# VictoriaMetrics/VictoriaLogs

Hardware: NVIDIA H100
Metric: log rows scanned/sec (LogsQL phrase+regex) (higher is better)
Workload: dtype u8

## Files before the change

### victorialogs_b200/csrc/vl_engine.cu

```cuda
#include <dlfcn.h>
#include <algorithm>
#include <atomic>
#include <chrono>
#include <cmath>
#include <limits>
#include <thread>
#include <cstdio>
#include <cstdlib>
#include <cstring>
#include <functional>
#include <map>
#include <memory>
#include <mutex>
#include "vl_copier.h"
#include "vl_engine.h"
#include "vl_kernels.cuh"
#include "vl_program.h"
#include "vl_part.h"
#include "vl_mathnum.cuh"

using namespace vl;

namespace vl {
static thread_local std::string g_thread_err;
// ... 47 lines not shown
}

namespace {

struct ZstdWriter {
    size_t (*compress)(void*, size_t, const void*, size_t, int) = nullptr;
    size_t (*bound)(size_t) = nullptr;
    unsigned (*is_error)(size_t) = nullptr;
    bool ok = false;
    ZstdWriter() {
        void* h = dlopen("libzstd.so.1", RTLD_NOW | RTLD_GLOBAL);
        if (!h) return;
        compress = (decltype(compress))dlsym(h, "ZSTD_compress");
        bound = (decltype(bound))dlsym(h, "ZSTD_compressBound");
        is_error = (decltype(is_error))dlsym(h, "ZSTD_isError");
        ok = compress && bound && is_error;
    }
};
ZstdWriter& zstd_writer() { static ZstdWriter z; return z; }

}

namespace vl {
void finish_batch_layout(vlscan_ctx* ctx, vlscan_batch* b, const std::vector<uint32_t>& rows) {
    b->nblocks = rows.size();
    b->h_rows = rows;
    b->h_word_off.assign(rows.size() + 1, 0);
    b->rows = 0;
    for (size_t i = 0; i < rows.size(); i++) { b->h_word_off[i + 1] = b->h_word_off[i] + (rows[i] + 63) / 64; b->rows += rows[i]; }
    b->nwords = b->h_word_off.back();
    std::vector<uint32_t> wb(b->nwords);
    std::vector<uint64_t> init(b->nwords);
    for (size_t i = 0; i < rows.size(); i++) {
        for (uint64_t w = b->h_word_off[i]; w < b->h_word_off[i + 1]; w++) { wb[w] = (uint32_t)i; init[w] = ~0ull; }
        uint32_t tail = rows[i] & 63;
        if (tail) init[b->h_word_off[i + 1] - 1] = (~0ull) >> (64 - tail);
    }
    b->blk_rows.ensure(std::max<size_t>(rows.size() * 4, 16));
    b->blk_word_off.ensure((rows.size() + 1) * 8);
    b->word_block.ensure(std::max<size_t>(b->nwords * 4, 16));
    b->init_bitmap.ensure(std::max<size_t>(b->nwords * 8, 16));
    if (!rows.empty()) VL_CUDA(cudaMemcpyAsync(b->blk_rows.p, rows.data(), rows.size() * 4, cudaMemcpyHostToDevice, ctx->stream));
    VL_CUDA(cudaMemcpyAsync(b->blk_word_off.p, b->h_word_off.data(), (rows.size() + 1) * 8, cudaMemcpyHostToDevice, ctx->stream));
    if (b->nwords) {
        VL_CUDA(cudaMemcpyAsync(b->word_block.p, wb.data(), b->nwords * 4, cudaMemcpyHostToDevice, ctx->stream));
        VL_CUDA(cudaMemcpyAsync(b->init_bitmap.p, init.data(), b->nwords * 8, cudaMemcpyHostToDevice, ctx->stream));
    }
    VL_CUDA(cudaStreamSynchronize(ctx->stream));
}
}

static uint64_t collect_values_blocks(const vlscan_block* blocks, uint64_t nblocks, std::vector<ZValuesBlock>& zv, const uint8_t* need = nullptr, uint32_t nfields = 0, std::vector<size_t>* at = nullptr) {
    uint64_t zc = 512;
    if (at) at->assign((size_t)nblocks * nfields, SIZE_MAX);
    for (uint64_t b = 0; b < nblocks; b++)
        for (uint32_t k = 0; k < blocks[b].ncols; k++) {
            const vlscan_column& c = blocks[b].cols[k];
            if (c.kind != VLSCAN_COL_VALUES || c.stage != VLSCAN_STAGE_ONDISK) continue;
            if (need && (c.field >= nfields || !need[b * nfields + c.field])) continue;
            if (at && c.field < nfields && (*at)[b * nfields + c.field] == SIZE_MAX) (*at)[b * nfields + c.field] = zv.size();
            zv.push_back({c.values, (size_t)c.values_len, zc});
            zc += c.values_len;
        }
    return zc;
}
static double now_s() { return std::chrono::duration<double>(std::chrono::steady_clock::now().time_since_epoch()).count(); }

namespace {
struct Upload {
    vlscan_ctx* ctx; vlscan_batch* out; const vlscan_block* blocks; uint64_t nblocks; uint32_t nfields; vlscan_stats* stats;
    const std::vector<char>* need_bloom;
    std::vector<DevColumn>& cols = out->h_cols;
    const bool dbg = getenv("VLSCAN_DEBUG_TIMING") != nullptr; const double t_start = now_s();
    Copier io{ctx};
    std::vector<uint32_t> rows = std::vector<uint32_t>(nblocks);
    std::vector<Piece> pieces;
    std::vector<std::unique_ptr<std::vector<uint8_t>>> owned;
    uint64_t cursor = 16;
    ZstdJob zjob;
    uint64_t regen_cursor = 0;
    struct Ondisk { uint64_t col; uint32_t lens_frame, data_frame; uint64_t lens_rel, data_rel; };
    std::vector<Ondisk> ondisk;
    std::vector<OndiskCol> ocols;
    struct TsFrame { uint64_t block; uint32_t frame; uint64_t rel; };
    std::vector<TsFrame> ts_frames;
    std::vector<DevTimestamps> tsv;
    std::vector<ZValuesBlock> zv; std::vector<ZValuesInfo> zinfo; std::vector<size_t> zv_of; std::vector<uint64_t> ts_zoff; size_t zbad = SIZE_MAX; std::string zmsg;
    uint64_t add_piece(const uint8_t* src, uint64_t len) { uint64_t off = arena_reserve(cursor, len); if (len) pieces.push_back({src, len, off}); return off; }
    template <class F> void walk(bool ts, F&& f) {
        for (uint64_t b = 0; b < nblocks; b++) {
            const vlscan_block& blk = blocks[b];
            if (blk.rows > (8u << 20)) throw BadInput("block rows exceed maxRowsPerBlock (8Mi)");
            rows[b] = (uint32_t)blk.rows;
            if (ts) timestamps(blk, b);
            for (uint32_t k = 0; k < blk.ncols; k++) {
                if (blk.cols[k].field >= nfields) throw BadInput("column refers to a field outside the batch field table");
                f(blk, blk.cols[k], (size_t)b * nfields + blk.cols[k].field);
            }
        }
    }
    void sources(const uint8_t* need, bool ts) {
        uint64_t zc = collect_values_blocks(blocks, nblocks, zv, need, nfields, &zv_of);
        for (const ZValuesBlock& v : zv) if (v.n) io.src.push_back({v.p, v.n, v.zoff});
        ts_zoff.resize(ts ? nblocks : 0);
        for (uint64_t b = 0; b < nblocks && ts; b++) {
            const vlscan_block& blk = blocks[b];
            if (blk.ts_marshal_type != MT_ZSTD_NEAREST_DELTA2 && blk.ts_marshal_type != MT_ZSTD_NEAREST_DELTA) continue;
            if (blk.timestamps_len > vl::part::kMaxTimestampsBlockSize) throw BadInput("timestamps block size cannot exceed 8 MiB");
            ts_zoff[b] = zc;
            if (blk.timestamps_len) io.src.push_back({blk.timestamps, blk.timestamps_len, zc});
            zc += blk.timestamps_len;
        }
        if (!io.src.empty()) { ctx->zsrc.ensure(zc + 512); io.send_sources(ctx->zsrc.as<uint8_t>()); }
        zinfo.resize(zv.size());
        const double t_w = now_s();
        if (!zv.empty()) zjob.add_values_blocks(zv.data(), zv.size(), host_threads(), zinfo.data(), &zbad, &zmsg);
        if (dbg) fprintf(stderr, "[vlscan upload] header walk of %zu values blocks on %d host threads: %.1f ms (after %.1f ms of collecting and enqueueing the copies)\n",
                         zv.size(), host_threads(), 1e3 * (now_s() - t_w), 1e3 * (t_w - t_start));
    }
    template <class F> void header(const vlscan_column& c, size_t i, F&& payload) {
        DevColumn& d = cols[i];
        if (d.kind != COL_MISSING) throw BadInput("duplicate column for one field in a block");
        if (c.kind == VLSCAN_COL_CONST) {
            d.kind = COL_CONST; d.meta_len = (uint32_t)c.const_len; d.meta_off = add_piece(c.const_value, c.const_len);
            return;
        }
        if (c.kind != VLSCAN_COL_VALUES) throw BadInput("unknown column kind");
        if (c.value_type < VT_STRING || c.value_type >= VT_MAX) throw BadInput("unknown valueType");
        d.kind = COL_VALUES; d.vt = c.value_type; d.min_value = c.min_value; d.max_value = c.max_value;
        payload();
        if (c.bloom_len % 8) throw BadInput("cannot unmarshal bloomFilter from src with size not multiple by 8");
        if (need_bloom && !(*need_bloom)[c.field]) { d.bloom_words = 0; d.bloom_off = add_piece(c.bloom, 0); }
        else { d.bloom_words = (uint32_t)(c.bloom_len / 8); d.bloom_off = add_piece(c.bloom, c.bloom_len); }
        if (c.value_type == VT_DICT) {
            if (c.dict_len > 8) throw BadInput("valuesDict may contain max 8 items");
            d.dict_len = c.dict_len;
            uint32_t total = c.dict_len ? c.dict_offsets[c.dict_len] : 0;
            d.meta_len = total;
            if (c.dict_len && c.dict_blob == (const uint8_t*)c.dict_offsets + 4 * (c.dict_len + 1)) {
// ... 34 lines not shown
            d.data_const = (blk.rows >= 2 && lt >= 4 && data_len == d.lens_const) ? 1 : 0;
        } else throw BadInput("unknown values stage");
    }
    void timestamps(const vlscan_block& blk, uint64_t b) {
        if (!blk.ts_marshal_type) return;
        if (blk.ts_marshal_type > MT_NEAREST_DELTA) throw BadInput("unknown MarshalType of a timestamps block");
        if (blk.timestamps_len > vl::part::kMaxTimestampsBlockSize) throw BadInput("timestamps block size cannot exceed 8 MiB");
        if (tsv.empty()) { tsv.resize(nblocks); memset(tsv.data(), 0, nblocks * sizeof(DevTimestamps)); }
        DevTimestamps& t = tsv[b];
        t.first = blk.min_timestamp; t.max = blk.max_timestamp;
        if (blk.ts_marshal_type == MT_ZSTD_NEAREST_DELTA2 || blk.ts_marshal_type == MT_ZSTD_NEAREST_DELTA) {
            uint64_t regen = 0; uint32_t id = 0;
            zjob.add_frame(blk.timestamps, blk.timestamps_len, ts_zoff[b], &regen, &id);
            if (regen > 10ull * blk.rows + 16) throw BadInput("cannot unmarshal timestamps: the decompressed block is larger than its varints can be");
            t.mt = blk.ts_marshal_type == MT_ZSTD_NEAREST_DELTA2 ? MT_NEAREST_DELTA2 : MT_NEAREST_DELTA;
            t.len = (uint32_t)regen;
            ts_frames.push_back({b, id, arena_reserve(regen_cursor, regen)});
        } else {
            t.mt = (uint8_t)blk.ts_marshal_type; t.len = (uint32_t)blk.timestamps_len;
            t.off = add_piece(blk.timestamps, blk.timestamps_len);
        }
    }

    uint64_t commit(DevBuf& region, const std::vector<uint64_t>* patch, bool layout) {
        const uint64_t regen_base = (cursor + kArenaAlign - 1) / kArenaAlign * kArenaAlign;
        for (const Ondisk& o : ondisk) {
            DevColumn& d = cols[o.col];
            d.lens_off += regen_base; d.data_off += regen_base;
            zjob.set_dst(o.lens_frame, regen_base + o.lens_rel); zjob.set_dst(o.data_frame, regen_base + o.data_rel);
        }
        for (const TsFrame& tf : ts_frames) { tsv[tf.block].off = regen_base + tf.rel; zjob.set_dst(tf.frame, regen_base + tf.rel); }
        const bool have_z = !ondisk.empty() || !ts_frames.empty();
        if (have_z) cursor = regen_base + regen_cursor;
        const uint64_t bytes = cursor + kArenaPad;
        const double t_desc = now_s();
        region.ensure(bytes);
        const double t_alloc = now_s();
        uint8_t* cols_base = region.as<uint8_t>();
        std::vector<ColPatch> patches;
        if (patch) {
            const uint64_t delta = (uint64_t)(uintptr_t)region.p - (uint64_t)(uintptr_t)out->arena.p;
            cols_base = out->arena.as<uint8_t>();
            patches.resize(patch->size());
            for (size_t i = 0; i < patch->size(); i++) {
                DevColumn& d = cols[(*patch)[i]];
                d.lens_off += delta; d.data_off += delta;
                patches[i].col = (*patch)[i]; patches[i].c = d;
            }
        }
        cudaStream_t cs = ctx->copy_stream;
        cudaEvent_t ev_cleared = io.events.make(), ev_copied = io.events.make();
        VL_CUDA(cudaMemsetAsync(region.p, 0, bytes, ctx->stream));
        VL_CUDA(cudaEventRecord(ev_cleared, ctx->stream));
        VL_CUDA(cudaStreamWaitEvent(cs, ev_cleared, 0));
        const double t_h2d = dbg ? now_s() : 0;
        double t_zrun = 0;
        if (have_z) {
            zjob.set_group_hook([&](uint64_t src_end) { io.wait_sources(ctx->stream, src_end); });
            zjob.run(ctx, ctx->zsrc.as<uint8_t>(), region.as<uint8_t>());
            io.ship_sources(UINT64_MAX);
            if (dbg) t_zrun = now_s();
        }
        io.copy(pieces, region.as<uint8_t>());
        DevBuf& table = patch ? ctx->patch : out->cols;
        const void* entries = patch ? (const void*)patches.data() : (const void*)cols.data();
        const size_t table_bytes = patch ? patches.size() * sizeof(ColPatch) : cols.size() * sizeof(DevColumn);
        table.ensure(std::max<size_t>(table_bytes, 16));
        if (table_bytes) VL_CUDA(cudaMemcpyAsync(table.p, entries, table_bytes, cudaMemcpyHostToDevice, cs));
        io.h2d += table_bytes;
        if (!patch) out->has_ts = !tsv.empty();
        if (!tsv.empty()) {
            out->ts.ensure(nblocks * sizeof(DevTimestamps));
            VL_CUDA(cudaMemcpyAsync(out->ts.p, tsv.data(), nblocks * sizeof(DevTimestamps), cudaMemcpyHostToDevice, cs));
            io.h2d += nblocks * sizeof(DevTimestamps);
        }
        VL_CUDA(cudaEventRecord(ev_copied, cs));
        if (!patches.empty()) {
            VL_CUDA(cudaStreamWaitEvent(ctx->stream, ev_copied, 0));
            k_patch_cols<<<cdiv(patches.size(), 128), 128, 0, ctx->stream>>>(out->cols.as<DevColumn>(), ctx->patch.as<ColPatch>(), (uint32_t)patches.size());
            launch_check(ctx);
        }
        const double t_enq = dbg ? now_s() : 0;
        if (have_z) {
            VL_CUDA(cudaStreamWaitEvent(ctx->stream, ev_copied, 0));
            ctx->zcols.ensure(16 + ocols.size() * sizeof(OndiskCol));
            VL_CUDA(cudaMemsetAsync(ctx->zcols.p, 0, 16, ctx->stream));
            VL_CUDA(cudaMemcpyAsync(ctx->zcols.as<uint8_t>() + 16, ocols.data(), ocols.size() * sizeof(OndiskCol), cudaMemcpyHostToDevice, ctx->stream));
            if (!ocols.empty()) {
                k_finish_ondisk_cols<<<cdiv(ocols.size(), 128), 128, 0, ctx->stream>>>(cols_base, out->cols.as<DevColumn>(), (const OndiskCol*)(ctx->zcols.as<uint8_t>() + 16),
                                                                                         (uint32_t)ocols.size(), ctx->zcols.as<unsigned long long>());
                launch_check(ctx);
            }
            io.h2d += ocols.size() * sizeof(OndiskCol);
            zjob.check(ctx);
            unsigned long long cst[2] = {0, 0};
            VL_CUDA(cudaMemcpy(cst, ctx->zcols.p, 16, cudaMemcpyDeviceToHost));
            static const char* what[] = {"", "cannot unmarshal uint64 block type from empty src", "unexpected uint64 block type", "unexpected block length for uint items", "row length does not fit 32 bits"};
            if (cst[0]) throw BadInput(what[std::min<unsigned long long>(cst[0], 4)]);
        }
        VL_CUDA(cudaStreamWaitEvent(ctx->stream, ev_copied, 0));
        double t_copy = 0;
        if (dbg) { VL_CUDA(cudaStreamSynchronize(ctx->stream)); t_copy = now_s(); }
        if (nfields) out->note_columns(cols);
        if (layout) finish_batch_layout(ctx, out, rows);
        else VL_CUDA(cudaStreamSynchronize(ctx->stream));
        if (dbg) fprintf(stderr, "[vlscan upload] blocks=%llu arena=%.1f MB h2d=%.1f MB pieces=%zu+%zu pinned=%d: describe %.1f ms, alloc %.1f ms, copy %.1f ms (%.1f GB/s), "
                                 "zstd %llu frames / %llu blocks / %llu sequences: enqueue %.1f ms, decode %.1f ms; layout %.1f ms\n", (unsigned long long)nblocks,
                         bytes / 1e6, io.h2d / 1e6, pieces.size(), io.src.size(), (int)io.all_pinned, 1e3 * (t_desc - t_start), 1e3 * (t_alloc - t_desc), 1e3 * (t_enq - (t_zrun > 0 ? t_zrun : t_h2d)), io.h2d / 1e9 / std::max(t_copy - t_start, 1e-9),
                         (unsigned long long)zjob.frames(), (unsigned long long)zjob.compressed_blocks(), (unsigned long long)zjob.sequences(), 1e3 * (t_zrun > 0 ? t_zrun - t_h2d : 0), 1e3 * (t_copy - t_enq), 1e3 * (now_s() - t_copy));
        if (layout) io.h2d += out->nwords * 12 + nblocks * 12;
        if (stats) stats->h2d_bytes += io.h2d;
        return bytes;
    }
};
}

enum UploadMode { UP_FULL = 0, UP_HEADERS = 1, UP_VALUES = 2, UP_LATE = 3 };
static void do_upload(vlscan_ctx* ctx, const char* const* field_names, const size_t* field_name_lens, uint32_t nfields, const vlscan_block* blocks,
                      uint64_t nblocks, vlscan_batch* out, vlscan_stats* stats, const std::vector<char>* need_bloom = nullptr, UploadMode mode = UP_FULL,
                      const uint8_t* need = nullptr, uint64_t* zframes = nullptr) {
    VL_CUDA(cudaSetDevice(ctx->device));
    if (nblocks > 0xFFFFFFF0ull) throw BadInput("too many blocks in one batch");
    out->device = ctx->device; out->nfields = nfields;
    Upload u{ctx, out, blocks, nblocks, nfields, stats, need_bloom};
    if (mode == UP_FULL || mode == UP_HEADERS) {
        for (uint32_t f = 0; f < nfields; f++) out->field_names.emplace_back(field_names[f], field_name_lens[f]);
        u.cols.assign((size_t)nblocks * std::max<uint32_t>(nfields, 1), DevColumn{});
        memset(u.cols.data(), 0, u.cols.size() * sizeof(DevColumn));
        out->late_used = 0; out->split_hdr = mode == UP_HEADERS;
    } else if (u.cols.size() != (size_t)nblocks * std::max<uint32_t>(nfields, 1) || !need) throw BadInput("internal: values phase of a bloom-first upload without its header phase");
    try {
        switch (mode) {
        case UP_FULL:
            u.sources(nullptr, true);
            u.walk(true, [&](const vlscan_block& blk, const vlscan_column& c, size_t i) { u.header(c, i, [&] { u.values(blk, c, i); }); });
            out->arena_bytes = u.commit(out->arena, nullptr, true);
            out->harena_bytes = 0;
            std::vector<DevColumn>().swap(out->h_cols);
            break;
        case UP_HEADERS:
            u.walk(false, [&](const vlscan_block&, const vlscan_column& c, size_t i) {
                u.header(c, i, [&] {
                    if (c.stage != VLSCAN_STAGE_ONDISK && c.stage != VLSCAN_STAGE_DECODED) throw BadInput("unknown values stage");
                    u.cols[i].values_state = VALUES_DEFERRED;
                });
            });
            out->harena_bytes = u.commit(out->harena, nullptr, true);
            break;
        case UP_VALUES:
            u.sources(need, true);
            u.walk(true, [&](const vlscan_block& blk, const vlscan_column& c, size_t i) {
                if (c.kind != VLSCAN_COL_VALUES) return;
                u.cols[i].values_state = need[i] ? VALUES_STAGED : VALUES_ABSENT;
                if (need[i]) u.values(blk, c, i);
            });
            out->arena_bytes = u.commit(out->arena, nullptr, false);
            break;
        case UP_LATE: {
            std::vector<uint64_t> staged;
            u.sources(need, false);
            u.walk(false, [&](const vlscan_block& blk, const vlscan_column& c, size_t i) {
                if (c.kind != VLSCAN_COL_VALUES || !need[i]) return;
                if (u.cols[i].values_state == VALUES_STAGED) throw BadInput("duplicate column for one field in a block");
                u.cols[i].values_state = VALUES_STAGED;
                u.values(blk, c, i);
                staged.push_back(i);
            });
            if (out->late_used == out->late.size()) out->late.emplace_back();
            u.commit(out->late[out->late_used], &staged, false);
            out->late_used++;
            *zframes += u.zjob.frames();
            break;
        }
        }
    } catch (...) {
        cudaStreamSynchronize(ctx->copy_stream); cudaStreamSynchronize(ctx->stream);
        throw;
    }
}

const uint32_t* vl::row_offsets(vlscan_ctx* ctx, const BatchView& B, int slot, const uint32_t* list, const uint32_t* wc, unsigned long long* stats, int wc_slot) {
    uint8_t* ready = ctx->ready[slot].as<uint8_t>();
    if (!ctx->ready_cleared[slot]) { VL_CUDA(cudaMemsetAsync(ready, 0, B.nblocks, ctx->stream)); ctx->ready_cleared[slot] = 1; }
    k_lens_offsets<<<ctx->sm_count * 8, 256, 0, ctx->stream>>>(B, slot, list, wc, ctx->row_off8[slot].as<uint32_t>(), ready, stats, wc_slot); launch_check(ctx);
    return ctx->row_off8[slot].as<uint32_t>();
}

namespace {
struct ScanRun {
    vlscan_ctx* ctx; const vlscan_program* prog; const vlscan_batch* batch;
    DevProgram P; BatchView B; std::vector<int> field_slot;
    unsigned long long* stats;
    size_t regs_used = 0;

    uint64_t* new_reg() {
        if (regs_used == ctx->regs.size()) ctx->regs.emplace_back();
        DevBuf& r = ctx->regs[regs_used++];
        r.ensure(std::max<size_t>(B.nwords * 8, 16));
        return r.as<uint64_t>();
    }
    void free_reg() { regs_used--; }
    void copy_reg(uint64_t* dst, const uint64_t* src) { if (B.nwords) VL_CUDA(cudaMemcpyAsync(dst, src, B.nwords * 8, cudaMemcpyDeviceToDevice, ctx->stream)); }
// ... 873 lines not shown
```

### victorialogs_b200/csrc/vl_zstd.cu

```cuda
#include "vl_zstd.h"

#include <algorithm>
#include <array>
#include <atomic>
#include <chrono>
#include <cstdio>
#include <cstdlib>
#include <cstring>
#include <exception>
#include <thread>

#include "vl_engine.h"
#include "vl_zstd.cuh"
#include "vl_zstd_job.h"

namespace vl {

using namespace zs;

struct ZstdDev {
    DevBuf frames, blocks, bstate, huf_tab, fse_tab, huf_state, fse_state, predef, lits, seqs, frame_err, status, lists;
    bool predef_ready = false;
    cudaStream_t xstream = nullptr;
    std::vector<cudaEvent_t> events;
    cudaEvent_t event(size_t i) {
        while (events.size() <= i) { cudaEvent_t e; VL_CUDA(cudaEventCreateWithFlags(&e, cudaEventDisableTiming)); events.push_back(e); }
        return events[i];
    }
    void* hpin = nullptr; size_t hpin_cap = 0;
    void* ensure_hpin(size_t n) {
        if (n <= hpin_cap) return hpin;
        if (hpin) cudaFreeHost(hpin);
        hpin = nullptr; hpin_cap = 0;
        VL_CUDA(cudaMallocHost(&hpin, n + n / 4 + 4096)); hpin_cap = n + n / 4 + 4096;
        return hpin;
    }
    void release() {
        DevBuf* all[] = {&frames, &blocks, &bstate, &huf_tab, &fse_tab, &huf_state, &fse_state, &predef, &lits, &seqs, &frame_err, &status, &lists};
        for (DevBuf* b : all) b->release();
        for (cudaEvent_t e : events) cudaEventDestroy(e);
        events.clear();
        if (xstream) cudaStreamDestroy(xstream);
        xstream = nullptr;
        if (hpin) cudaFreeHost(hpin);
        hpin = nullptr; hpin_cap = 0;
    }
};

static __global__ void k_pull_words(uint4* __restrict__ dst, const uint4* __restrict__ src, size_t n) {
    for (size_t i = (size_t)blockIdx.x * blockDim.x + threadIdx.x; i < n; i += (size_t)gridDim.x * blockDim.x) dst[i] = src[i];
}
void zstd_dev_free(ZstdDev* d) { if (d) { d->release(); delete d; } }

namespace {
inline unsigned cdiv_u(uint64_t a, uint64_t b) { return (unsigned)((a + b - 1) / b); }
}

struct ZstdJob::Impl : ZstdJobImpl {};

ZstdJob::ZstdJob() : m(new Impl) {}
ZstdJob::~ZstdJob() { delete m; }
bool ZstdJob::empty() const { return m->frames.empty(); }
uint64_t ZstdJob::frames() const { return m->frames.size(); }
uint64_t ZstdJob::blocks() const { return m->blocks.size(); }
uint64_t ZstdJob::compressed_blocks() const { return m->n_compressed; }
uint64_t ZstdJob::sequences() const { return m->n_seqs; }
// ... 31 lines not shown
                dry.add_bytes_block(v[i].p + c1, v[i].n - c1, v[i].zoff + c1, &r, &id);
            } catch (const BadInput&) { break; }
        }
        total_seqs = dry.m->n_seqs;
    }
    auto taper = [&] { if (!group_scale_env()) m->limit_scale = (m->groups.empty() || m->n_seqs > total_seqs - total_seqs / 12) ? 1 : 4; };
    for (size_t i = 0; i < n; i++) {
        try {
            uint32_t f1 = 0, f2 = 0;
            taper();
            const size_t c1 = add_bytes_block(v[i].p, v[i].n, v[i].zoff, &info[i].lens_len, &f1);
            taper();
            const size_t c2 = add_bytes_block(v[i].p + c1, v[i].n - c1, v[i].zoff + c1, &info[i].data_len, &f2);
            if (c1 + c2 != v[i].n) throw BadInput("unexpected non-empty tail after reading bytes block with strings");
        } catch (const BadInput& e) { *bad = i; *msg = e.msg; return; }
    }
    if (!group_scale_env()) m->limit_scale = 1;
}

void ZstdJob::prepare() { m->prepare(); }

void ZstdJob::digest(uint64_t out[4]) const { m->digest(out); }

void ZstdJob::run(vlscan_ctx* ctx, const uint8_t* zsrc, uint8_t* arena) {
    Impl& J = *m;
    if (J.frames.empty()) return;
    auto now = [] { return std::chrono::duration<double>(std::chrono::steady_clock::now().time_since_epoch()).count(); };
    const double t_prep = now();
    J.prepare();
    const double t_lists = now();
    const std::vector<uint32_t>& lists = J.lists;
    if (!ctx->zdev) ctx->zdev = new ZstdDev;
    ZstdDev& D = *ctx->zdev;
    cudaStream_t st = ctx->stream;
    D.frames.ensure(J.frames.size() * sizeof(ZFrame) + 16); D.blocks.ensure(J.blocks.size() * sizeof(ZBlock) + 16); D.bstate.ensure(J.blocks.size() * sizeof(ZBlockState));
    D.frame_err.ensure(J.frames.size() * 4); D.status.ensure(16); D.lists.ensure(lists.size() * 4 + 16);
    D.huf_tab.ensure(std::max<size_t>((size_t)J.max_huf * Z_HUF_TABLE * 2, 16)); D.huf_state.ensure(std::max<size_t>((size_t)J.max_huf * sizeof(ZSlotState), 16));
    D.fse_tab.ensure(std::max<size_t>((size_t)J.max_fse * Z_FSE_SLOT_BYTES, 16)); D.fse_state.ensure(std::max<size_t>((size_t)J.max_fse * sizeof(ZSlotState), 16));
    const size_t lits_stride = (J.max_lits + 64 + 255) / 256 * 256, seqs_stride = std::max<size_t>(J.max_seqs, 1);
    D.lits.ensure(2 * lits_stride); D.seqs.ensure(2 * seqs_stride * 16);
    if (!D.xstream) VL_CUDA(cudaStreamCreateWithFlags(&D.xstream, cudaStreamNonBlocking));
    if (!D.predef_ready) {
        D.predef.ensure(Z_FSE_SLOT_BYTES);
        k_zstd_predef<<<1, 32, 0, st>>>(D.predef.as<uint8_t>());
        VL_CUDA(cudaFuncSetAttribute(k_seq_decode, cudaFuncAttributeMaxDynamicSharedMemorySize, (int)(Z_SEQ_CTA_LANES * (Z_FSE_SLOT_BYTES + Z_LINEBUF))));
        VL_CUDA(cudaFuncSetAttribute(k_huf_decode, cudaFuncAttributeMaxDynamicSharedMemorySize, (int)(Z_HUF_CTA_BLOCKS * Z_HUF_TABLE * 2)));
        ctx->launches++; VL_CUDA(cudaGetLastError());
        D.predef_ready = true;
    }
    {
        auto up16 = [](size_t n) { return (n + 15) / 16 * 16; };
        const size_t nf = up16(J.frames.size() * sizeof(ZFrame)), nb = up16(J.blocks.size() * sizeof(ZBlock)), nl = up16(lists.size() * 4);
        uint8_t* h = (uint8_t*)D.ensure_hpin(nf + nb + nl + 64);
        const double t_cp = now();
        J.spread_copy(h, J.frames.data(), J.frames.size() * sizeof(ZFrame));
        J.spread_copy(h + nf, J.blocks.data(), J.blocks.size() * sizeof(ZBlock));
        if (!lists.empty()) J.spread_copy(h + nf + nb, lists.data(), lists.size() * 4);
        if (getenv("VLSCAN_DEBUG_TIMING")) fprintf(stderr, "[vlscan zstd] host: work lists of %zu launch groups %.1f ms, %.1f MB of tables to pinned memory %.1f ms (%d threads)\n",
                                                   J.groups.size(), 1e3 * (t_lists - t_prep), (nf + nb + nl) / 1e6, 1e3 * (now() - t_cp), std::max(J.threads, 1));
        k_pull_words<<<296, 256, 0, st>>>(D.frames.as<uint4>(), (const uint4*)h, nf / 16); ctx->launches++;
        k_pull_words<<<296, 256, 0, st>>>(D.blocks.as<uint4>(), (const uint4*)(h + nf), nb / 16); ctx->launches++;
        if (nl) { k_pull_words<<<296, 256, 0, st>>>(D.lists.as<uint4>(), (const uint4*)(h + nf + nb), nl / 16); ctx->launches++; }
        VL_CUDA(cudaGetLastError());
    }
    VL_CUDA(cudaMemsetAsync(D.frame_err.p, 0, J.frames.size() * 4, st));
    VL_CUDA(cudaMemsetAsync(D.status.p, 0, 16, st));
    VL_CUDA(cudaMemsetAsync(D.bstate.p, 0, J.blocks.size() * sizeof(ZBlockState), st));
    ZView V{};
    V.src = zsrc; V.arena = arena; V.frames = D.frames.as<ZFrame>(); V.blocks = D.blocks.as<ZBlock>(); V.bstate = D.bstate.as<ZBlockState>();
    V.huf_tab = D.huf_tab.as<uint16_t>(); V.fse_tab = D.fse_tab.as<uint8_t>(); V.huf_state = D.huf_state.as<ZSlotState>(); V.fse_state = D.fse_state.as<ZSlotState>();
    V.predef = D.predef.as<uint8_t>(); V.lits = D.lits.as<uint8_t>(); V.seqs = D.seqs.as<uint4>(); V.frame_err = D.frame_err.as<unsigned int>();
    V.status = D.status.as<unsigned long long>();
    const uint32_t* L = D.lists.as<uint32_t>();
    const bool dbg = getenv("VLSCAN_DEBUG_TIMING") != nullptr;
    static const char* phase_name[6] = {"huf_build", "huf_decode", "fse_build", "seq_decode", "seq_resolve", "execute"};
    std::vector<std::pair<int, std::pair<cudaEvent_t, cudaEvent_t>>> marks;
    int phase = 0;
    static const bool overlap = [] { const char* e = getenv("VLSCAN_ZSTD_OVERLAP"); return !e || atoi(e) != 0; }();
    cudaStream_t xs = overlap ? D.xstream : st;
    cudaStream_t cur_stream = st;
    auto begin = [&](int p) { phase = p; if (dbg) { cudaEvent_t a, b; cudaEventCreate(&a); cudaEventCreate(&b); cudaEventRecord(a, cur_stream); marks.push_back({p, {a, b}}); } };
    auto launched = [&] { ctx->launches++; VL_CUDA(cudaGetLastError()); if (dbg) cudaEventRecord(marks.back().second.second, cur_stream); };
    VL_CUDA(cudaEventRecord(D.event(0), st)); VL_CUDA(cudaStreamWaitEvent(xs, D.event(0), 0));
    size_t gi = 0;
    for (const Group& g : J.groups) {
        uint32_t nh = g.huf_hi - g.huf_lo, nl = g.lit_hi - g.lit_lo, ns = g.seq_hi - g.seq_lo, nf = g.frame_hi - g.frame_lo;
        if (J.group_hook) {
            uint64_t need = 0;
            for (uint32_t i = J.frames[g.frame_lo].blk_lo; i < J.frames[g.frame_hi - 1].blk_hi; i++) need = std::max<uint64_t>(need, J.blocks[i].src + (J.blocks[i].type == ZB_RLE ? 1 : J.blocks[i].size));
            J.group_hook(need);
        }
        ZView W = V;
        W.lits = V.lits + (gi & 1) * lits_stride; W.seqs = V.seqs + (gi & 1) * seqs_stride;
        cudaEvent_t ev_entropy = D.event(1 + 2 * gi), ev_exec = D.event(2 + 2 * gi);
        cur_stream = st;
// ... 6 lines not shown
        }
        VL_CUDA(cudaEventRecord(ev_entropy, st));
        VL_CUDA(cudaStreamWaitEvent(xs, ev_entropy, 0));
        cur_stream = xs;
        begin(4); k_seq_resolve<<<cdiv_u(nf, 64), 64, 0, xs>>>(W, g.frame_lo, nf); launched();
        begin(5); k_execute<<<cdiv_u((uint64_t)nf * 32, Z_EXEC_WARPS * 32), Z_EXEC_WARPS * 32, 0, xs>>>(W, L + g.ord_lo, nf); launched();
        VL_CUDA(cudaEventRecord(ev_exec, xs));
        gi++;
    }
    if (gi) VL_CUDA(cudaStreamWaitEvent(st, D.event(2 + 2 * (gi - 1)), 0));
    cur_stream = st;
    if (dbg) {
        VL_CUDA(cudaStreamSynchronize(xs)); VL_CUDA(cudaStreamSynchronize(st));
        float tot[6] = {0, 0, 0, 0, 0, 0};
        for (auto& mk : marks) { float ms = 0; cudaEventElapsedTime(&ms, mk.second.first, mk.second.second); tot[mk.first] += ms; cudaEventDestroy(mk.second.first); cudaEventDestroy(mk.second.second); }
        fprintf(stderr, "[vlscan zstd] %zu groups:", J.groups.size());
        for (int p = 0; p < 6; p++) fprintf(stderr, " %s %.2f ms", phase_name[p], tot[p]);
        fprintf(stderr, "\n");
    }
    (void)phase;
    J.ran = true;
}

void ZstdJob::check(vlscan_ctx* ctx) {
    if (!m->ran) return;
    unsigned long long stt[2] = {0, 0};
    VL_CUDA(cudaMemcpyAsync(stt, ctx->zdev->status.p, 16, cudaMemcpyDeviceToHost, ctx->stream));
    VL_CUDA(cudaStreamSynchronize(ctx->stream));
    if (!stt[0]) return;
    static const char* what[] = {"", "bad Huffman tree description", "bad Huffman stream", "bad FSE table description", "bad sequences bitstream", "match offset beyond the regenerated data",
                                 "regenerated size differs from the frame content size", "bad literals section"};
    throw BadInput(std::string("cannot decompress block: ") + (stt[0] < 8 ? what[stt[0]] : "corrupted frame") + " (frame " + std::to_string(stt[1] - 1) + " of the batch)");
}

}
```

### victorialogs_b200/csrc/vl_zstd.h

```cpp
#pragma once
#include <stddef.h>
#include <stdint.h>
#include <functional>
#include <string>
#include <vector>

struct vlscan_ctx;

namespace vl {

struct ZstdDev;
void zstd_dev_free(ZstdDev* d);

struct ZstdTimings { float total_ms = 0; };

struct ZValuesBlock { const uint8_t* p; size_t n; uint64_t zoff; };
struct ZValuesInfo { uint64_t lens_len, data_len; };

class ZstdJob {
public:
    ZstdJob();
    ~ZstdJob();
    ZstdJob(const ZstdJob&) = delete;
    ZstdJob& operator=(const ZstdJob&) = delete;
    size_t add_bytes_block(const uint8_t* p, size_t n, uint64_t zoff, uint64_t* regen, uint32_t* id);
    void add_frame(const uint8_t* f, size_t n, uint64_t zoff, uint64_t* regen, uint32_t* id);
    void add_values_blocks(const ZValuesBlock* v, size_t n, int threads, ZValuesInfo* info, size_t* bad, std::string* msg);
    void prepare();
    void digest(uint64_t out[4]) const;
    void set_dst(uint32_t id, uint64_t arena_off);
    bool empty() const;
    uint64_t frames() const;
    uint64_t blocks() const;
    uint64_t compressed_blocks() const;
    uint64_t sequences() const;
    uint64_t groups() const;
    void set_group_hook(std::function<void(uint64_t src_end)> f);
    void run(vlscan_ctx* ctx, const uint8_t* zsrc, uint8_t* arena);
    void check(vlscan_ctx* ctx);
private:
    struct Impl;
    Impl* m;
};

}
```

### victorialogs_b200/csrc/vl_zstd_job.h

```cpp
#pragma once
#include <stddef.h>
#include <stdint.h>
#include <stdlib.h>
#include <string.h>
#include <algorithm>
#include <array>
#include <atomic>
#include <exception>
#include <functional>
#include <string>
#include <thread>
#include <vector>
#include "vl_zstd.h"
#include "vl_zstd_types.h"
#include "vl_zstd_walk.h"

namespace vl {

using namespace zs;

inline uint64_t group_scale_env() { static const uint64_t v = [] { const char* e = getenv("VLSCAN_ZSTD_GROUP_SCALE"); long x = e ? atol(e) : 0; return (uint64_t)(x < 0 ? 0 : x > 64 ? 64 : x); }(); return v; }
static const uint64_t kGroupLitsUnit = 512ull << 20, kGroupSeqsUnit = 64ull << 20;
static const uint32_t kGroupSlotsUnit = 32u << 10;

struct Group { uint32_t frame_lo, frame_hi; uint32_t huf_lo, huf_hi, lit_lo, lit_hi, seq_lo, seq_hi, ord_lo, ord_hi; };

struct FrameUse { uint64_t lits, seqs; uint32_t huf, fse; };

struct ZstdJobImpl {
    std::vector<ZFrame> frames;
    std::vector<ZBlock> blocks;
    std::vector<Group> groups;
    std::vector<uint32_t> lists;
    uint64_t g_lits = 0, g_seqs = 0; uint32_t g_huf = 0, g_fse = 0; uint32_t g_frame_lo = 0;
    uint64_t limit_scale = group_scale_env() ? group_scale_env() : 4;
    uint64_t max_lits = 0, max_seqs = 0; uint32_t max_huf = 0, max_fse = 0;
    uint64_t n_compressed = 0, n_seqs = 0;
    int threads = 0;
    bool prepared = false, ran = false;
    std::function<void(uint64_t)> group_hook;

    void close_group_at(uint32_t f) {
        if (g_frame_lo == f) return;
        Group g{}; g.frame_lo = g_frame_lo; g.frame_hi = f;
        groups.push_back(g);
        max_lits = std::max(max_lits, g_lits); max_seqs = std::max(max_seqs, g_seqs); max_huf = std::max(max_huf, g_huf); max_fse = std::max(max_fse, g_fse);
        g_lits = g_seqs = 0; g_huf = g_fse = 0; g_frame_lo = f;
    }
    void close_group() { close_group_at((uint32_t)frames.size()); }

    static FrameUse frame_use(const ZBlock* b, uint32_t cnt) {
        FrameUse u{0, 0, 0, 0};
        for (uint32_t i = 0; i < cnt; i++) {
            if (b[i].type != ZB_COMPRESSED) continue;
            if (b[i].lit_type >= ZL_COMPRESSED) u.lits += b[i].lit_regen;
            u.seqs += b[i].nseq; u.huf += b[i].huf_own != Z_PREDEF; u.fse += b[i].fse_own != Z_PREDEF;
        }
        return u;
    }
    FrameUse admit_frame(uint32_t f, const FrameUse& u) {
        const uint64_t m = limit_scale;
        if (g_frame_lo != f && (g_lits + u.lits > kGroupLitsUnit * m || g_seqs + u.seqs > kGroupSeqsUnit * m || g_huf + u.huf > kGroupSlotsUnit * m || g_fse + u.fse > kGroupSlotsUnit * m)) close_group_at(f);
// ... 167 lines not shown
```

### victorialogs_b200/csrc/vl_zstd_walk.h

```cpp
#pragma once
#include <stddef.h>
#include <stdint.h>
#include <algorithm>
#include <string>
#include <vector>
#include "vl_zstd_types.h"

namespace vl {

struct BadInput { std::string msg; explicit BadInput(std::string m) : msg(std::move(m)) {} };

namespace zwalk {

using namespace zs;

const uint32_t kNone = 0xFFFFFFFEu;
const uint64_t kMaxFrameContent = 1ull << 30;
const uint32_t kBlockMax = 128u << 10;

inline uint32_t le16(const uint8_t* p) { return p[0] | (p[1] << 8); }
inline uint32_t le24(const uint8_t* p) { return p[0] | (p[1] << 8) | (p[2] << 16); }
inline uint32_t le32(const uint8_t* p) { return p[0] | (p[1] << 8) | (p[2] << 16) | ((uint32_t)p[3] << 24); }
inline uint64_t le40(const uint8_t* p) { return (uint64_t)le32(p) | ((uint64_t)p[4] << 32); }
inline uint64_t le64(const uint8_t* p) { return (uint64_t)le32(p) | ((uint64_t)le32(p + 4) << 32); }
// ... 94 lines not shown
    if (p[0] == 0) {
        if (n < 2) throw BadInput("cannot unmarshal plain block size from empty src");
        size_t len = p[1];
        if (n - 2 < len) throw BadInput("cannot read plain block: not enough bytes");
        ZFrame fr{}; fr.fcs = len; fr.blk_lo = (uint32_t)blocks.size();
        ZBlock B{}; B.src = zoff + 2; B.size = (uint32_t)len; B.frame = fid; B.type = ZB_RAW;
        B.huf_own = B.huf_slot = B.fse_own = B.ll_slot = B.of_slot = B.ml_slot = Z_PREDEF;
        blocks.push_back(B);
        fr.blk_hi = (uint32_t)blocks.size();
        out = fr;
        return 2 + len;
    }
    if (p[0] == 1) {
        uint64_t clen = 0; int sh = 0; size_t i = 1; bool done = false;
        for (; i < n && i < 11; i++) { clen |= (uint64_t)(p[i] & 0x7F) << sh; sh += 7; if (p[i] < 0x80) { done = true; i++; break; } }
        if (!done) throw BadInput("cannot unmarshal compressed block size");
        if (n - i < clen) throw BadInput("cannot read compressed block: not enough bytes");
        parse_frame_into(blocks, fid, p + i, clen, zoff + i, out);
        return i + clen;
    }
    throw BadInput("unexpected block type; supported types: 0, 1");
}

}
}
```

Before: 22.70 billion.

## Split zstd values decode into two jobs and overlap host layout with decoding

For large uploads the values blocks are split: the first sixth has a full header walk up front, while the rest only gets a cheap frame-header peek for content sizes. That remainder is fully walked and decoded as a second job after the first is launched, so host parsing overlaps GPU decoding. Batch layout construction on the host now runs while the decoder is in flight, and only the upload waits. Adds per-job status slots, a pinned-buffer reuse event and a retry without splitting on decode errors, at the cost of extra complexity and a possible double upload on bad input.

```diff
diff --git a/victorialogs_b200/csrc/vl_engine.cu b/victorialogs_b200/csrc/vl_engine.cu
--- a/victorialogs_b200/csrc/vl_engine.cu
+++ b/victorialogs_b200/csrc/vl_engine.cu
@@ -93,20 +93,24 @@
 }
 
 namespace vl {
-void finish_batch_layout(vlscan_ctx* ctx, vlscan_batch* b, const std::vector<uint32_t>& rows) {
+struct BatchLayout { std::vector<uint32_t> wb; std::vector<uint64_t> init; };
+static void build_batch_layout(vlscan_batch* b, const std::vector<uint32_t>& rows, BatchLayout& L) {
     b->nblocks = rows.size();
     b->h_rows = rows;
     b->h_word_off.assign(rows.size() + 1, 0);
     b->rows = 0;
     for (size_t i = 0; i < rows.size(); i++) { b->h_word_off[i + 1] = b->h_word_off[i] + (rows[i] + 63) / 64; b->rows += rows[i]; }
     b->nwords = b->h_word_off.back();
-    std::vector<uint32_t> wb(b->nwords);
-    std::vector<uint64_t> init(b->nwords);
+    std::vector<uint32_t>& wb = L.wb; std::vector<uint64_t>& init = L.init;
+    wb.resize(b->nwords); init.resize(b->nwords);
     for (size_t i = 0; i < rows.size(); i++) {
         for (uint64_t w = b->h_word_off[i]; w < b->h_word_off[i + 1]; w++) { wb[w] = (uint32_t)i; init[w] = ~0ull; }
         uint32_t tail = rows[i] & 63;
         if (tail) init[b->h_word_off[i + 1] - 1] = (~0ull) >> (64 - tail);
     }
+}
+static void upload_batch_layout(vlscan_ctx* ctx, vlscan_batch* b, const BatchLayout& L) {
+    const std::vector<uint32_t>& rows = b->h_rows; const std::vector<uint32_t>& wb = L.wb; const std::vector<uint64_t>& init = L.init;
     b->blk_rows.ensure(std::max<size_t>(rows.size() * 4, 16));
     b->blk_word_off.ensure((rows.size() + 1) * 8);
     b->word_block.ensure(std::max<size_t>(b->nwords * 4, 16));
@@ -118,6 +122,11 @@
         VL_CUDA(cudaMemcpyAsync(b->init_bitmap.p, init.data(), b->nwords * 8, cudaMemcpyHostToDevice, ctx->stream));
     }
     VL_CUDA(cudaStreamSynchronize(ctx->stream));
+}
+void finish_batch_layout(vlscan_ctx* ctx, vlscan_batch* b, const std::vector<uint32_t>& rows) {
+    BatchLayout L;
+    build_batch_layout(b, rows, L);
+    upload_batch_layout(ctx, b, L);
 }
 }
 
@@ -138,6 +147,7 @@
 static double now_s() { return std::chrono::duration<double>(std::chrono::steady_clock::now().time_since_epoch()).count(); }
 
 namespace {
+static const size_t kSplitValuesBlocks = 4096;
 struct Upload {
     vlscan_ctx* ctx; vlscan_batch* out; const vlscan_block* blocks; uint64_t nblocks; uint32_t nfields; vlscan_stats* stats;
     const std::vector<char>* need_bloom;
@@ -150,6 +160,9 @@
     uint64_t cursor = 16;
     ZstdJob zjob;
     uint64_t regen_cursor = 0;
+    bool split = false;
+    ZstdJob zjob2;
+    size_t z_split = 0;
     struct Ondisk { uint64_t col; uint32_t lens_frame, data_frame; uint64_t lens_rel, data_rel; };
     std::vector<Ondisk> ondisk;
     std::vector<OndiskCol> ocols;
@@ -185,7 +198,23 @@
         if (!io.src.empty()) { ctx->zsrc.ensure(zc + 512); io.send_sources(ctx->zsrc.as<uint8_t>()); }
         zinfo.resize(zv.size());
         const double t_w = now_s();
-        if (!zv.empty()) zjob.add_values_blocks(zv.data(), zv.size(), host_threads(), zinfo.data(), &zbad, &zmsg);
+        if (split && zv.size() >= kSplitValuesBlocks && host_threads() > 0) {
+            const size_t lo = zv.size() / 6, n = zv.size() - lo;
+            const int T = std::max(1, host_threads());
+            std::atomic<bool> ok{true};
+            auto peek = [&](int t) {
+                for (size_t z = lo + n * (size_t)t / T; z < lo + n * (size_t)(t + 1) / T; z++) {
+                    size_t u1 = 0, u2 = 0;
+                    if (!zwalk::peek_bytes_block(zv[z].p, zv[z].n, &zinfo[z].lens_len, &u1) || !zwalk::peek_bytes_block(zv[z].p + u1, zv[z].n - u1, &zinfo[z].data_len, &u2) || u1 + u2 != zv[z].n) { ok = false; return; }
+                }
+            };
+            std::vector<std::thread> pool;
+            for (int t = 1; t < T; t++) pool.emplace_back(peek, t);
+            peek(0);
+            for (auto& th : pool) th.join();
+            z_split = ok ? lo : 0;
+        }
+        if (!zv.empty()) zjob.add_values_blocks(zv.data(), z_split ? z_split : zv.size(), host_threads(), zinfo.data(), &zbad, &zmsg);
         if (dbg) fprintf(stderr, "[vlscan upload] header walk of %zu values blocks on %d host threads: %.1f ms (after %.1f ms of collecting and enqueueing the copies)\n",
                          zv.size(), host_threads(), 1e3 * (now_s() - t_w), 1e3 * (t_w - t_start));
     }
@@ -266,11 +295,24 @@
         }
     }
 
+    void decode_check() {
+        unsigned long long a[2], b[2] = {0, 0};
+        zjob.status(ctx, a);
+        if (z_split) zjob2.status(ctx, b);
+        if (!a[0] && !b[0]) return;
+        const uint64_t nz = zv.size();
+        auto global_a = [&](uint64_t f) { return f < 2 * z_split ? f : 2 * nz + (f - 2 * z_split); };
+        uint64_t frame = 0;
+        if (a[0]) frame = std::max<uint64_t>(frame, z_split ? global_a(a[1] - 1) : a[1] - 1);
+        if (b[0]) frame = std::max<uint64_t>(frame, 2 * z_split + (b[1] - 1));
+        throw BadInput(ZstdJob::status_message(std::max(a[0], b[0]), frame));
+    }
     uint64_t commit(DevBuf& region, const std::vector<uint64_t>* patch, bool layout) {
         const uint64_t regen_base = (cursor + kArenaAlign - 1) / kArenaAlign * kArenaAlign;
         for (const Ondisk& o : ondisk) {
             DevColumn& d = cols[o.col];
             d.lens_off += regen_base; d.data_off += regen_base;
+            if (o.lens_frame >= 2 * z_split && z_split) continue;
             zjob.set_dst(o.lens_frame, regen_base + o.lens_rel); zjob.set_dst(o.data_frame, regen_base + o.data_rel);
         }
         for (const TsFrame& tf : ts_frames) { tsv[tf.block].off = regen_base + tf.rel; zjob.set_dst(tf.frame, regen_base + tf.rel); }
@@ -301,7 +343,20 @@
         double t_zrun = 0;
         if (have_z) {
             zjob.set_group_hook([&](uint64_t src_end) { io.wait_sources(ctx->stream, src_end); });
-            zjob.run(ctx, ctx->zsrc.as<uint8_t>(), region.as<uint8_t>());
+            zjob.run(ctx, ctx->zsrc.as<uint8_t>(), region.as<uint8_t>(), 0);
+            if (z_split) {
+                const size_t n2 = zv.size() - z_split;
+                std::vector<ZValuesInfo> info2(n2);
+                size_t bad2 = SIZE_MAX; std::string msg2;
+                zjob2.add_values_blocks(zv.data() + z_split, n2, host_threads(), info2.data(), &bad2, &msg2);
+                if (bad2 != SIZE_MAX) throw BadInput(msg2);
+                for (size_t i = 0; i < n2; i++)
+                    if (info2[i].lens_len != zinfo[z_split + i].lens_len || info2[i].data_len != zinfo[z_split + i].data_len) throw BadInput("internal: a frame header walk disagrees with its content size");
+                for (const Ondisk& o : ondisk)
+                    if (o.lens_frame >= 2 * z_split) { zjob2.set_dst(o.lens_frame - 2 * z_split, regen_base + o.lens_rel); zjob2.set_dst(o.data_frame - 2 * z_split, regen_base + o.data_rel); }
+                zjob2.set_group_hook([&](uint64_t src_end) { io.wait_sources(ctx->stream, src_end); });
+                zjob2.run(ctx, ctx->zsrc.as<uint8_t>(), region.as<uint8_t>(), 1);
+            }
             io.ship_sources(UINT64_MAX);
             if (dbg) t_zrun = now_s();
         }
@@ -324,6 +379,10 @@
             k_patch_cols<<<cdiv(patches.size(), 128), 128, 0, ctx->stream>>>(out->cols.as<DevColumn>(), ctx->patch.as<ColPatch>(), (uint32_t)patches.size());
             launch_check(ctx);
         }
+        const double t_host = dbg ? now_s() : 0;
+        if (nfields) out->note_columns(cols);
+        BatchLayout lay;
+        if (layout) build_batch_layout(out, rows, lay);
         const double t_enq = dbg ? now_s() : 0;
         if (have_z) {
             VL_CUDA(cudaStreamWaitEvent(ctx->stream, ev_copied, 0));
@@ -336,7 +395,7 @@
                 launch_check(ctx);
             }
             io.h2d += ocols.size() * sizeof(OndiskCol);
-            zjob.check(ctx);
+            decode_check();
             unsigned long long cst[2] = {0, 0};
             VL_CUDA(cudaMemcpy(cst, ctx->zcols.p, 16, cudaMemcpyDeviceToHost));
             static const char* what[] = {"", "cannot unmarshal uint64 block type from empty src", "unexpected uint64 block type", "unexpected block length for uint items", "row length does not fit 32 bits"};
@@ -345,13 +404,12 @@
         VL_CUDA(cudaStreamWaitEvent(ctx->stream, ev_copied, 0));
         double t_copy = 0;
         if (dbg) { VL_CUDA(cudaStreamSynchronize(ctx->stream)); t_copy = now_s(); }
-        if (nfields) out->note_columns(cols);
-        if (layout) finish_batch_layout(ctx, out, rows);
+        if (layout) upload_batch_layout(ctx, out, lay);
         else VL_CUDA(cudaStreamSynchronize(ctx->stream));
         if (dbg) fprintf(stderr, "[vlscan upload] blocks=%llu arena=%.1f MB h2d=%.1f MB pieces=%zu+%zu pinned=%d: describe %.1f ms, alloc %.1f ms, copy %.1f ms (%.1f GB/s), "
-                                 "zstd %llu frames / %llu blocks / %llu sequences: enqueue %.1f ms, decode %.1f ms; layout %.1f ms\n", (unsigned long long)nblocks,
-                         bytes / 1e6, io.h2d / 1e6, pieces.size(), io.src.size(), (int)io.all_pinned, 1e3 * (t_desc - t_start), 1e3 * (t_alloc - t_desc), 1e3 * (t_enq - (t_zrun > 0 ? t_zrun : t_h2d)), io.h2d / 1e9 / std::max(t_copy - t_start, 1e-9),
-                         (unsigned long long)zjob.frames(), (unsigned long long)zjob.compressed_blocks(), (unsigned long long)zjob.sequences(), 1e3 * (t_zrun > 0 ? t_zrun - t_h2d : 0), 1e3 * (t_copy - t_enq), 1e3 * (now_s() - t_copy));
+                                 "zstd %llu frames / %llu blocks / %llu sequences: enqueue %.1f ms, host layout beside the decoder %.1f ms, decode %.1f ms; layout upload %.1f ms\n", (unsigned long long)nblocks,
+                         bytes / 1e6, io.h2d / 1e6, pieces.size(), io.src.size(), (int)io.all_pinned, 1e3 * (t_desc - t_start), 1e3 * (t_alloc - t_desc), 1e3 * (t_host - (t_zrun > 0 ? t_zrun : t_h2d)), io.h2d / 1e9 / std::max(t_copy - t_start, 1e-9),
+                         (unsigned long long)zjob.frames(), (unsigned long long)zjob.compressed_blocks(), (unsigned long long)zjob.sequences(), 1e3 * (t_zrun > 0 ? t_zrun - t_h2d : 0), 1e3 * (t_enq - t_host), 1e3 * (t_copy - t_enq), 1e3 * (now_s() - t_copy));
         if (layout) io.h2d += out->nwords * 12 + nblocks * 12;
         if (stats) stats->h2d_bytes += io.h2d;
         return bytes;
@@ -360,9 +418,9 @@
 }
 
 enum UploadMode { UP_FULL = 0, UP_HEADERS = 1, UP_VALUES = 2, UP_LATE = 3 };
-static void do_upload(vlscan_ctx* ctx, const char* const* field_names, const size_t* field_name_lens, uint32_t nfields, const vlscan_block* blocks,
-                      uint64_t nblocks, vlscan_batch* out, vlscan_stats* stats, const std::vector<char>* need_bloom = nullptr, UploadMode mode = UP_FULL,
-                      const uint8_t* need = nullptr, uint64_t* zframes = nullptr) {
+static void do_upload_once(vlscan_ctx* ctx, const char* const* field_names, const size_t* field_name_lens, uint32_t nfields, const vlscan_block* blocks,
+                           uint64_t nblocks, vlscan_batch* out, vlscan_stats* stats, const std::vector<char>* need_bloom, UploadMode mode,
+                           const uint8_t* need, uint64_t* zframes, bool split, bool* was_split) {
     VL_CUDA(cudaSetDevice(ctx->device));
     if (nblocks > 0xFFFFFFF0ull) throw BadInput("too many blocks in one batch");
     out->device = ctx->device; out->nfields = nfields;
@@ -376,7 +434,9 @@
     try {
         switch (mode) {
         case UP_FULL:
+            u.split = split;
             u.sources(nullptr, true);
+            *was_split = u.z_split != 0;
             u.walk(true, [&](const vlscan_block& blk, const vlscan_column& c, size_t i) { u.header(c, i, [&] { u.values(blk, c, i); }); });
             out->arena_bytes = u.commit(out->arena, nullptr, true);
             out->harena_bytes = 0;
@@ -422,6 +482,21 @@
         throw;
     }
 }
+static void do_upload(vlscan_ctx* ctx, const char* const* field_names, const size_t* field_name_lens, uint32_t nfields, const vlscan_block* blocks,
+                      uint64_t nblocks, vlscan_batch* out, vlscan_stats* stats, const std::vector<char>* need_bloom = nullptr, UploadMode mode = UP_FULL,
+                      const uint8_t* need = nullptr, uint64_t* zframes = nullptr) {
+    bool was_split = false;
+    const size_t nnames = out->field_names.size();
+    const vlscan_stats saved = stats ? *stats : vlscan_stats{};
+    try {
+        do_upload_once(ctx, field_names, field_name_lens, nfields, blocks, nblocks, out, stats, need_bloom, mode, need, zframes, mode == UP_FULL, &was_split);
+    } catch (const BadInput&) {
+        if (!was_split) throw;
+        out->field_names.resize(nnames);
+        if (stats) *stats = saved;
+        do_upload_once(ctx, field_names, field_name_lens, nfields, blocks, nblocks, out, stats, need_bloom, mode, need, zframes, false, &was_split);
+    }
+}
 
 const uint32_t* vl::row_offsets(vlscan_ctx* ctx, const BatchView& B, int slot, const uint32_t* list, const uint32_t* wc, unsigned long long* stats, int wc_slot) {
     uint8_t* ready = ctx->ready[slot].as<uint8_t>();
diff --git a/victorialogs_b200/csrc/vl_zstd.cu b/victorialogs_b200/csrc/vl_zstd.cu
--- a/victorialogs_b200/csrc/vl_zstd.cu
+++ b/victorialogs_b200/csrc/vl_zstd.cu
@@ -23,6 +23,7 @@
     bool predef_ready = false;
     cudaStream_t xstream = nullptr;
     std::vector<cudaEvent_t> events;
+    cudaEvent_t pulled = nullptr;
     cudaEvent_t event(size_t i) {
         while (events.size() <= i) { cudaEvent_t e; VL_CUDA(cudaEventCreateWithFlags(&e, cudaEventDisableTiming)); events.push_back(e); }
         return events[i];
@@ -42,6 +43,8 @@
         events.clear();
         if (xstream) cudaStreamDestroy(xstream);
         xstream = nullptr;
+        if (pulled) cudaEventDestroy(pulled);
+        pulled = nullptr;
         if (hpin) cudaFreeHost(hpin);
         hpin = nullptr; hpin_cap = 0;
     }
@@ -119,7 +122,7 @@
 
 void ZstdJob::digest(uint64_t out[4]) const { m->digest(out); }
 
-void ZstdJob::run(vlscan_ctx* ctx, const uint8_t* zsrc, uint8_t* arena) {
+void ZstdJob::run(vlscan_ctx* ctx, const uint8_t* zsrc, uint8_t* arena, int slot) {
     Impl& J = *m;
     if (J.frames.empty()) return;
     auto now = [] { return std::chrono::duration<double>(std::chrono::steady_clock::now().time_since_epoch()).count(); };
@@ -131,7 +134,7 @@
     ZstdDev& D = *ctx->zdev;
     cudaStream_t st = ctx->stream;
     D.frames.ensure(J.frames.size() * sizeof(ZFrame) + 16); D.blocks.ensure(J.blocks.size() * sizeof(ZBlock) + 16); D.bstate.ensure(J.blocks.size() * sizeof(ZBlockState));
-    D.frame_err.ensure(J.frames.size() * 4); D.status.ensure(16); D.lists.ensure(lists.size() * 4 + 16);
+    D.frame_err.ensure(J.frames.size() * 4); D.status.ensure(16 * kStatusSlots); D.lists.ensure(lists.size() * 4 + 16);
     D.huf_tab.ensure(std::max<size_t>((size_t)J.max_huf * Z_HUF_TABLE * 2, 16)); D.huf_state.ensure(std::max<size_t>((size_t)J.max_huf * sizeof(ZSlotState), 16));
     D.fse_tab.ensure(std::max<size_t>((size_t)J.max_fse * Z_FSE_SLOT_BYTES, 16)); D.fse_state.ensure(std::max<size_t>((size_t)J.max_fse * sizeof(ZSlotState), 16));
     const size_t lits_stride = (J.max_lits + 64 + 255) / 256 * 256, seqs_stride = std::max<size_t>(J.max_seqs, 1);
@@ -148,6 +151,8 @@
     {
         auto up16 = [](size_t n) { return (n + 15) / 16 * 16; };
         const size_t nf = up16(J.frames.size() * sizeof(ZFrame)), nb = up16(J.blocks.size() * sizeof(ZBlock)), nl = up16(lists.size() * 4);
+        if (D.pulled) VL_CUDA(cudaEventSynchronize(D.pulled));
+        else VL_CUDA(cudaEventCreateWithFlags(&D.pulled, cudaEventDisableTiming));
         uint8_t* h = (uint8_t*)D.ensure_hpin(nf + nb + nl + 64);
         const double t_cp = now();
         J.spread_copy(h, J.frames.data(), J.frames.size() * sizeof(ZFrame));
@@ -159,15 +164,17 @@
         k_pull_words<<<296, 256, 0, st>>>(D.blocks.as<uint4>(), (const uint4*)(h + nf), nb / 16); ctx->launches++;
         if (nl) { k_pull_words<<<296, 256, 0, st>>>(D.lists.as<uint4>(), (const uint4*)(h + nf + nb), nl / 16); ctx->launches++; }
         VL_CUDA(cudaGetLastError());
+        VL_CUDA(cudaEventRecord(D.pulled, st));
     }
     VL_CUDA(cudaMemsetAsync(D.frame_err.p, 0, J.frames.size() * 4, st));
-    VL_CUDA(cudaMemsetAsync(D.status.p, 0, 16, st));
+    VL_CUDA(cudaMemsetAsync(D.status.as<uint8_t>() + 16 * slot, 0, 16, st));
     VL_CUDA(cudaMemsetAsync(D.bstate.p, 0, J.blocks.size() * sizeof(ZBlockState), st));
     ZView V{};
     V.src = zsrc; V.arena = arena; V.frames = D.frames.as<ZFrame>(); V.blocks = D.blocks.as<ZBlock>(); V.bstate = D.bstate.as<ZBlockState>();
     V.huf_tab = D.huf_tab.as<uint16_t>(); V.fse_tab = D.fse_tab.as<uint8_t>(); V.huf_state = D.huf_state.as<ZSlotState>(); V.fse_state = D.fse_state.as<ZSlotState>();
     V.predef = D.predef.as<uint8_t>(); V.lits = D.lits.as<uint8_t>(); V.seqs = D.seqs.as<uint4>(); V.frame_err = D.frame_err.as<unsigned int>();
-    V.status = D.status.as<unsigned long long>();
+    V.status = D.status.as<unsigned long long>() + 2 * slot;
+    J.slot = slot;
     const uint32_t* L = D.lists.as<uint32_t>();
     const bool dbg = getenv("VLSCAN_DEBUG_TIMING") != nullptr;
     static const char* phase_name[6] = {"huf_build", "huf_decode", "fse_build", "seq_decode", "seq_resolve", "execute"};
@@ -220,15 +227,23 @@
     J.ran = true;
 }
 
-void ZstdJob::check(vlscan_ctx* ctx) {
+void ZstdJob::status(vlscan_ctx* ctx, unsigned long long out[2]) const {
+    out[0] = out[1] = 0;
     if (!m->ran) return;
-    unsigned long long stt[2] = {0, 0};
-    VL_CUDA(cudaMemcpyAsync(stt, ctx->zdev->status.p, 16, cudaMemcpyDeviceToHost, ctx->stream));
+    VL_CUDA(cudaMemcpyAsync(out, ctx->zdev->status.as<unsigned long long>() + 2 * m->slot, 16, cudaMemcpyDeviceToHost, ctx->stream));
     VL_CUDA(cudaStreamSynchronize(ctx->stream));
-    if (!stt[0]) return;
+}
+
+std::string ZstdJob::status_message(unsigned long long code, unsigned long long frame) {
     static const char* what[] = {"", "bad Huffman tree description", "bad Huffman stream", "bad FSE table description", "bad sequences bitstream", "match offset beyond the regenerated data",
                                  "regenerated size differs from the frame content size", "bad literals section"};
-    throw BadInput(std::string("cannot decompress block: ") + (stt[0] < 8 ? what[stt[0]] : "corrupted frame") + " (frame " + std::to_string(stt[1] - 1) + " of the batch)");
-}
-
-}
+    return std::string("cannot decompress block: ") + (code < 8 ? what[code] : "corrupted frame") + " (frame " + std::to_string(frame) + " of the batch)";
+}
+
+void ZstdJob::check(vlscan_ctx* ctx) {
+    unsigned long long stt[2];
+    status(ctx, stt);
+    if (stt[0]) throw BadInput(status_message(stt[0], stt[1] - 1));
+}
+
+}
diff --git a/victorialogs_b200/csrc/vl_zstd.h b/victorialogs_b200/csrc/vl_zstd.h
--- a/victorialogs_b200/csrc/vl_zstd.h
+++ b/victorialogs_b200/csrc/vl_zstd.h
@@ -36,7 +36,10 @@
     uint64_t sequences() const;
     uint64_t groups() const;
     void set_group_hook(std::function<void(uint64_t src_end)> f);
-    void run(vlscan_ctx* ctx, const uint8_t* zsrc, uint8_t* arena);
+    static const int kStatusSlots = 2;
+    void run(vlscan_ctx* ctx, const uint8_t* zsrc, uint8_t* arena, int slot = 0);
+    void status(vlscan_ctx* ctx, unsigned long long out[2]) const;
+    static std::string status_message(unsigned long long code, unsigned long long frame);
     void check(vlscan_ctx* ctx);
 private:
     struct Impl;
diff --git a/victorialogs_b200/csrc/vl_zstd_job.h b/victorialogs_b200/csrc/vl_zstd_job.h
--- a/victorialogs_b200/csrc/vl_zstd_job.h
+++ b/victorialogs_b200/csrc/vl_zstd_job.h
@@ -38,6 +38,7 @@
     uint64_t n_compressed = 0, n_seqs = 0;
     int threads = 0;
     bool prepared = false, ran = false;
+    int slot = 0;
     std::function<void(uint64_t)> group_hook;
 
     void close_group_at(uint32_t f) {
diff --git a/victorialogs_b200/csrc/vl_zstd_walk.h b/victorialogs_b200/csrc/vl_zstd_walk.h
--- a/victorialogs_b200/csrc/vl_zstd_walk.h
+++ b/victorialogs_b200/csrc/vl_zstd_walk.h
@@ -140,5 +140,25 @@
     throw BadInput("unexpected block type; supported types: 0, 1");
 }
 
+inline bool peek_bytes_block(const uint8_t* p, size_t n, uint64_t* regen, size_t* used) {
+    if (n < 2) return false;
+    if (p[0] == 0) { if (n - 2 < p[1]) return false; *regen = p[1]; *used = 2 + (size_t)p[1]; return true; }
+    if (p[0] != 1) return false;
+    uint64_t clen = 0; int sh = 0; size_t i = 1; bool done = false;
+    for (; i < n && i < 11; i++) { clen |= (uint64_t)(p[i] & 0x7F) << sh; sh += 7; if (p[i] < 0x80) { done = true; i++; break; } }
+    if (!done || n - i < clen) return false;
+    const uint8_t* f = p + i;
+    if (clen < 6 || le32(f) != 0xFD2FB528u) return false;
+    const uint32_t fhd = f[4], fcs_flag = fhd >> 6, single = (fhd >> 5) & 1, did_flag = fhd & 3;
+    if ((fhd & 8) || did_flag) return false;
+    const size_t pos = single ? 5 : 6;
+    const int fcs_sz = fcs_flag == 0 ? (single ? 1 : 0) : fcs_flag == 1 ? 2 : fcs_flag == 2 ? 4 : 8;
+    if (!fcs_sz || pos + fcs_sz > clen) return false;
+    const uint64_t fcs = fcs_sz == 1 ? f[pos] : fcs_sz == 2 ? le16(f + pos) + 256u : fcs_sz == 4 ? le32(f + pos) : le64(f + pos);
+    if (fcs > kMaxFrameContent) return false;
+    *regen = fcs; *used = i + clen;
+    return true;
+}
+
 }
 }
```

Result: no change. 22.71 billion, median of 6 (+0.0%).
